# TaceoLabs/co-snarks

Hardware: NVIDIA H100
Metric: co-Groth16 proofs/sec (BN254, 2^20 constraints); MSM Mscalar/s (higher is better)
Workload: dtype u32x8 (256-bit Montgomery, integer)

## Files before the change

### co_snarks_b200/csrc/cs_curve.cuh

```cuda
#pragma once
#include "cs_field.cuh"

namespace cs {

template <class P>
struct Fp2 {
  typedef Fp<P> F;
  static constexpr int N = 2 * P::N;
  F c0, c1;
  static CS_D Fp2 zero() { Fp2 r; r.c0 = F::zero(); r.c1 = F::zero(); return r; }
  static CS_D Fp2 one() { Fp2 r; r.c0 = F::one(); r.c1 = F::zero(); return r; }
  CS_D bool is_zero() const { return c0.is_zero() && c1.is_zero(); }
  CS_D bool operator==(const Fp2& b) const { return c0 == b.c0 && c1 == b.c1; }
  CS_D bool operator!=(const Fp2& b) const { return !(*this == b); }
  friend CS_D Fp2 operator+(const Fp2& a, const Fp2& b) { Fp2 r; r.c0 = a.c0 + b.c0; r.c1 = a.c1 + b.c1; return r; }
  friend CS_D Fp2 operator-(const Fp2& a, const Fp2& b) { Fp2 r; r.c0 = a.c0 - b.c0; r.c1 = a.c1 - b.c1; return r; }
  friend CS_D Fp2 operator*(const Fp2& a, const Fp2& b) { return mul_ool(a, b); }
  static CS_DN Fp2 mul_ool(Fp2 a, Fp2 b) {
    constexpr int W = 2 * P::N;
    uint32_t v0[W], v1[W], v2[W];
    F::mul_wide(v0, a.c0, b.c0);
    F::mul_wide(v1, a.c1, b.c1);
    F::mul_wide(v2, F::add_unreduced(a.c0, a.c1), F::add_unreduced(b.c0, b.c1));
    sub_n<W>(v2, v0);
    sub_n<W>(v2, v1);
    add_mod_sq<P, 1>(v0);
    sub_n<W>(v0, v1);
    Fp2 r;
    r.c0 = F::redc(v0);
    r.c1 = F::redc(v2);
    return r;
  }
  static CS_DN Fp2 mul_sub_ool(Fp2 a, Fp2 b, Fp2 c, Fp2 d) {
    constexpr int W = 2 * P::N;
    uint32_t t0[W], t1[W], t[W];
    CS_UNROLL
    for (int i = 0; i < W; i++) t0[i] = t1[i] = mod_sq<P, 2>(i);
    F::mul_wide(t, a.c0, b.c0);
    add_n<W>(t0, t);
    sub_n<W>(t1, t);
    F::mul_wide(t, a.c1, b.c1);
    sub_n<W>(t0, t);
    sub_n<W>(t1, t);
    F::mul_wide(t, F::add_unreduced(a.c0, a.c1), F::add_unreduced(b.c0, b.c1));
    add_n<W>(t1, t);
    F::mul_wide(t, c.c0, d.c0);
    sub_n<W>(t0, t);
    add_n<W>(t1, t);
    F::mul_wide(t, c.c1, d.c1);
    add_n<W>(t0, t);
    add_n<W>(t1, t);
    F::mul_wide(t, F::add_unreduced(c.c0, c.c1), F::add_unreduced(d.c0, d.c1));
    sub_n<W>(t1, t);
    Fp2 r;
    r.c0 = F::redc(t0);
    r.c1 = F::redc(t1);
    return r;
  }
  CS_D Fp2 sqr() const { return sqr_ool(*this); }
  static CS_DN Fp2 sqr_ool(Fp2 a) {
    Fp2 r;
    F t = F::mul_inline(a.c0, a.c1);
    r.c0 = F::mul_inline(a.c0 + a.c1, a.c0 - a.c1);
    r.c1 = t + t;
    return r;
  }
  CS_D Fp2 neg() const { Fp2 r; r.c0 = c0.neg(); r.c1 = c1.neg(); return r; }
  CS_D Fp2 dbl() const { Fp2 r; r.c0 = c0.dbl(); r.c1 = c1.dbl(); return r; }
  CS_D Fp2 inverse() const {
    F n = (c0.sqr() + c1.sqr()).inverse();
    Fp2 r;
    r.c0 = c0 * n;
    r.c1 = (c1 * n).neg();
    return r;
  }
};

template <class P>
CS_D Fp<P> mul_sub(const Fp<P>& a, const Fp<P>& b, const Fp<P>& c, const Fp<P>& d) { return Fp<P>::dot2(a, b, c.neg(), d); }
template <class P>
CS_D Fp2<P> mul_sub(const Fp2<P>& a, const Fp2<P>& b, const Fp2<P>& c, const Fp2<P>& d) {
  return Fp2<P>::mul_sub_ool(a, b, c, d);
}

template <class F>
struct Affine {
  F x, y;
  CS_D bool is_inf() const { return x.is_zero() && y.is_zero(); }
  static CS_D Affine inf() { Affine r; r.x = F::zero(); r.y = F::zero(); return r; }
};

template <class F>
struct Xyzz {
  F x, y, zz, zzz;
  CS_D bool is_inf() const { return zz.is_zero(); }
  static CS_D Xyzz inf() {
    Xyzz r;
    r.x = F::zero(); r.y = F::zero(); r.zz = F::zero(); r.zzz = F::zero();
    return r;
  }
  static CS_D Xyzz from_affine(const Affine<F>& p) {
    if (p.is_inf()) return inf();
    Xyzz r;
    r.x = p.x; r.y = p.y; r.zz = F::one(); r.zzz = F::one();
    return r;
  }
};

template <class F>
CS_DN Xyzz<F> dbl_affine(const Affine<F>& p) {
  Xyzz<F> r;
  if (p.y.is_zero()) return Xyzz<F>::inf();
  F U = p.y.dbl();
  F V = U.sqr();
  F W = U * V;
  F S = p.x * V;
  F X2 = p.x.sqr();
  F M = X2.dbl() + X2;
  r.x = M.sqr() - S.dbl();
  r.y = mul_sub(M, S - r.x, W, p.y);
  r.zz = V;
  r.zzz = W;
  return r;
}

template <class F>
CS_DN Xyzz<F> dbl_xyzz(const Xyzz<F>& p) {
  if (p.is_inf() || p.y.is_zero()) return Xyzz<F>::inf();
  Xyzz<F> r;
  F U = p.y.dbl();
  F V = U.sqr();
  F W = U * V;
  F S = p.x * V;
  F X2 = p.x.sqr();
  F M = X2.dbl() + X2;
  r.x = M.sqr() - S.dbl();
  r.y = mul_sub(M, S - r.x, W, p.y);
  r.zz = V * p.zz;
  r.zzz = W * p.zzz;
  return r;
}

template <class F>
CS_D void madd(Xyzz<F>& acc, const Affine<F>& p_in, bool negate) {
  if (p_in.is_inf()) return;
  Affine<F> p = p_in;
  if (negate) p.y = p.y.neg();
  if (acc.is_inf()) {
    acc.x = p.x; acc.y = p.y; acc.zz = F::one(); acc.zzz = F::one();
    return;
  }
  F U2 = p.x * acc.zz;
  F S2 = p.y * acc.zzz;
  F Pp = U2 - acc.x;
  F R = S2 - acc.y;
  if (Pp.is_zero()) {
    if (R.is_zero()) acc = dbl_affine(p);
    else acc = Xyzz<F>::inf();
    return;
  }
  F PP = Pp.sqr();
  F PPP = Pp * PP;
  F Q = acc.x * PP;
  F X3 = R.sqr() - PPP - Q.dbl();
  acc.y = mul_sub(R, Q - X3, acc.y, PPP);
  acc.x = X3;
  acc.zz = acc.zz * PP;
  acc.zzz = acc.zzz * PPP;
}

template <class F>
CS_D void padd(Xyzz<F>& acc, const Xyzz<F>& q) {
  if (q.is_inf()) return;
  if (acc.is_inf()) { acc = q; return; }
  F U1 = acc.x * q.zz;
  F U2 = q.x * acc.zz;
  F S1 = acc.y * q.zzz;
  F S2 = q.y * acc.zzz;
  F Pp = U2 - U1;
  F R = S2 - S1;
  if (Pp.is_zero()) {
    if (R.is_zero()) acc = dbl_xyzz(acc);
    else acc = Xyzz<F>::inf();
    return;
  }
  F PP = Pp.sqr();
  F PPP = Pp * PP;
  F Q = U1 * PP;
  F X3 = R.sqr() - PPP - Q.dbl();
  acc.y = mul_sub(R, Q - X3, S1, PPP);
  acc.x = X3;
  acc.zz = acc.zz * q.zz * PP;
  acc.zzz = acc.zzz * q.zzz * PPP;
}

template <class P>
CS_D Fp<P> shfl_down(const Fp<P>& a, unsigned delta) {
  Fp<P> r;
#if defined(CS_EMU)
  cs::emu::shfl_bytes(&a, &r, sizeof(r), 1, delta);
  return r;
#endif
  CS_UNROLL
  for (int i = 0; i < P::N; i++) r.l[i] = __shfl_down_sync(0xffffffffu, a.l[i], delta);
  return r;
}
template <class P>
CS_D Fp2<P> shfl_down(const Fp2<P>& a, unsigned delta) {
  Fp2<P> r;
  r.c0 = shfl_down(a.c0, delta);
  r.c1 = shfl_down(a.c1, delta);
  return r;
}
template <class F>
CS_D Xyzz<F> shfl_down(const Xyzz<F>& p, unsigned delta) {
  Xyzz<F> r;
#if defined(CS_EMU)
  cs::emu::shfl_bytes(&p, &r, sizeof(r), 1, delta);
  return r;
#endif
  r.x = shfl_down(p.x, delta); r.y = shfl_down(p.y, delta);
  r.zz = shfl_down(p.zz, delta); r.zzz = shfl_down(p.zzz, delta);
  return r;
}

template <class F>
CS_DN Affine<F> to_affine(const Xyzz<F>& p) {
  if (p.is_inf()) return Affine<F>::inf();
  F zi = p.zzz.inverse();
  F zzi = (zi * p.zz).sqr();
  Affine<F> r;
  r.x = p.x * zzi;
  r.y = p.y * zi;
  return r;
}

}
```

### co_snarks_b200/csrc/cs_msm.cuh

```cuda
#pragma once
#include <stdlib.h>
#include "cs_common.cuh"
#include "cs_curve.cuh"

namespace cs {

constexpr unsigned MSM_SLICE_MAX = 64;
constexpr unsigned MSM_ORDER_BLOCK = 256;
constexpr unsigned MSM_RED_SEG = 4;
constexpr unsigned MSM_SIGN = 0x80000000u;

template <class FrP, class Fn>
CS_D void msm_recode(const uint32_t* __restrict__ scalars, uint32_t sstride, uint32_t i, int mont, uint32_t c,
                     uint32_t W, uint32_t k, Fn&& f) {
  Fp<FrP> s;
  const uint4* src = reinterpret_cast<const uint4*>(scalars) + (size_t)i * sstride * (FrP::N / 4);
  CS_UNROLL
  for (int q = 0; q < FrP::N / 4; q++) {
    uint4 v = src[q];
    s.l[4 * q] = v.x; s.l[4 * q + 1] = v.y; s.l[4 * q + 2] = v.z; s.l[4 * q + 3] = v.w;
  }
  if (mont) s = s.from_mont();
  const uint32_t half = 1u << (c - 1);
  const uint32_t mask = (1u << c) - 1;
  uint32_t carry = 0, row = 0, gb = 0;
  for (uint32_t w = 0; w < W; w++) {
    uint32_t pos = w * c;
    uint32_t li = pos >> 5, sh = pos & 31;
    uint32_t lo = li < FrP::N ? s.l[li] : 0;
    uint32_t hi = li + 1 < FrP::N ? s.l[li + 1] : 0;
    uint32_t d = (__funnelshift_r(lo, hi, sh) & mask) + carry;
    uint32_t out;
    if (d > half) {
      out = ((1u << c) - d) | MSM_SIGN;
      carry = 1;
    } else {
      out = d;
      carry = 0;
    }
    f(row, out & ~MSM_SIGN ? out + gb : 0);
    gb += half;
    if (gb == k * half) {
      gb = 0;
      row++;
    }
  }
}

CS_D bool msm_base_inf(const uint32_t* __restrict__ infmask, uint32_t k) {
  return infmask && ((infmask[k >> 5] >> (k & 31)) & 1);
}

constexpr unsigned MSM_BIN_T = 1024;
constexpr unsigned MSM_BIN_TILE = 4096;
constexpr unsigned MSM_BIN_SPAN = 1u << 15;
constexpr unsigned MSM_SCATTER_SPAN = 1u << 13;

template <class FrP>
CS_GLOBAL void __launch_bounds__(MSM_BIN_T) k_msm_bin_count(const uint32_t* __restrict__ scalars, uint32_t sstride,
                                                            uint32_t n, int mont, uint32_t c, uint32_t W, uint32_t kw,
                                                            const uint32_t* __restrict__ infmask, uint32_t offset,
                                                            uint32_t tile, uint32_t B, uint32_t* __restrict__ tab) {
  CS_DYN_SMEM(uint32_t, h);
  const uint32_t lo = blockIdx.y * MSM_BIN_SPAN + 1;
  const uint32_t span = B + 1 - lo < MSM_BIN_SPAN ? B + 1 - lo : MSM_BIN_SPAN;
  for (uint32_t k = threadIdx.x; k < span; k += blockDim.x) h[k] = 0;
  __syncthreads();
  const uint32_t i1 = (blockIdx.x + 1) * tile < n ? (blockIdx.x + 1) * tile : n;
  for (uint32_t i = blockIdx.x * tile + threadIdx.x; i < i1; i += blockDim.x) {
    if (msm_base_inf(infmask, offset + i)) continue;
    msm_recode<FrP>(scalars, sstride, i, mont, c, W, kw, [&](uint32_t, uint32_t d) {
      const uint32_t k = (d & ~MSM_SIGN) - lo;
      if (k < span) atomicAdd(&h[k], 1u);
    });
  }
  __syncthreads();
  uint32_t* row = tab + (size_t)blockIdx.x * B + (lo - 1);
  for (uint32_t k = threadIdx.x; k < span; k += blockDim.x) row[k] = h[k];
}

constexpr unsigned MSM_BIN_SCAN_U = 16;
static CS_GLOBAL void k_msm_bin_scan(uint32_t* __restrict__ tab, uint32_t nblk, uint32_t B, uint32_t* __restrict__ count) {
  const uint32_t b = blockIdx.x * blockDim.x + threadIdx.x;
  if (b == 0) count[0] = 0;
  if (b >= B) return;
  uint32_t* col = tab + b;
  uint32_t run = 0, r = 0;
  for (; r + MSM_BIN_SCAN_U <= nblk; r += MSM_BIN_SCAN_U) {
    uint32_t v[MSM_BIN_SCAN_U];
    CS_UNROLL
    for (uint32_t u = 0; u < MSM_BIN_SCAN_U; u++) v[u] = col[(size_t)(r + u) * B];
    CS_UNROLL
    for (uint32_t u = 0; u < MSM_BIN_SCAN_U; u++) {
      col[(size_t)(r + u) * B] = run;
      run += v[u];
    }
  }
  for (; r < nblk; r++) {
    const uint32_t v = col[(size_t)r * B];
    col[(size_t)r * B] = run;
    run += v;
  }
  count[b + 1] = run;
}

template <class FrP>
CS_GLOBAL void __launch_bounds__(MSM_BIN_T) k_msm_bin_scatter(const uint32_t* __restrict__ scalars, uint32_t sstride,
                                                              uint32_t n, int mont, uint32_t c, uint32_t W, uint32_t kw,
                                                              const uint32_t* __restrict__ infmask, uint32_t offset,
                                                              uint32_t tile, uint32_t B, uint32_t nbases,
                                                              const uint32_t* __restrict__ tab,
                                                              const uint32_t* __restrict__ start,
                                                              uint32_t* __restrict__ sorted) {
  CS_DYN_SMEM(uint32_t, cur);
  const uint32_t lo = blockIdx.y * MSM_SCATTER_SPAN + 1;
  const uint32_t span = B + 1 - lo < MSM_SCATTER_SPAN ? B + 1 - lo : MSM_SCATTER_SPAN;
  const uint32_t* row = tab + (size_t)blockIdx.x * B + (lo - 1);
  for (uint32_t k = threadIdx.x; k < span; k += blockDim.x) cur[k] = start[lo + k] + row[k];
  __syncthreads();
  const uint32_t i1 = (blockIdx.x + 1) * tile < n ? (blockIdx.x + 1) * tile : n;
  for (uint32_t i = blockIdx.x * tile + threadIdx.x; i < i1; i += blockDim.x) {
    if (msm_base_inf(infmask, offset + i)) continue;
    msm_recode<FrP>(scalars, sstride, i, mont, c, W, kw, [&](uint32_t row, uint32_t d) {
      const uint32_t k = (d & ~MSM_SIGN) - lo;
      if (k < span) sorted[atomicAdd(&cur[k], 1u)] = (row * nbases + offset + i) | (d & MSM_SIGN);
    });
  }
}

template <class F>
CS_GLOBAL void k_msm_infmask(const Affine<F>* __restrict__ table, uint32_t n, uint32_t* __restrict__ mask) {
  uint32_t wd = blockIdx.x * blockDim.x + threadIdx.x;
  if (wd * 32 >= n) return;
  uint32_t m = 0;
  for (uint32_t k = 0; k < 32 && wd * 32 + k < n; k++)
    if (table[wd * 32 + k].is_inf()) m |= 1u << k;
  mask[wd] = m;
}

constexpr unsigned MSM_SCAN_T = 1024;
constexpr unsigned MSM_SCAN_MAX_BLOCKS = 1024;
CS_D void msm_scan_terms(const uint32_t* __restrict__ count, uint32_t k, uint32_t nb1, uint32_t S, uint32_t* v) {
  uint32_t cnt = (k && k < nb1) ? count[k] : 0;
  uint32_t n0 = (cnt + S - 1) / S;
  uint32_t n1 = (n0 + S - 1) / S;
  v[0] = cnt; v[1] = n0; v[2] = n1; v[3] = (n1 + S - 1) / S;
}
static CS_GLOBAL void k_msm_scan1(const uint32_t* __restrict__ count, uint32_t nb1 , uint32_t S,
                                  uint32_t* __restrict__ start, uint32_t* __restrict__ sstart0,
                                  uint32_t* __restrict__ sstart1, uint32_t* __restrict__ sstart2, uint32_t* __restrict__ aux) {
  __shared__ uint32_t sm[4][32];
  const uint32_t t = threadIdx.x, lane = t & 31, wid = t >> 5, nwarp = blockDim.x >> 5;
  const uint32_t k = blockIdx.x * blockDim.x + t;
  uint32_t v[4], inc[4];
  msm_scan_terms(count, k, nb1, S, v);
  CS_UNROLL
  for (int q = 0; q < 4; q++) {
    uint32_t x = v[q];
    CS_UNROLL
    for (uint32_t d = 1; d < 32; d <<= 1) {
      uint32_t y = __shfl_up_sync(0xffffffffu, x, d);
      if (lane >= d) x += y;
    }
    inc[q] = x;
    if (lane == 31) sm[q][wid] = x;
  }
  __syncthreads();
  uint32_t w[4], x[4];
  CS_UNROLL
  for (int q = 0; q < 4; q++) {
    w[q] = (wid == 0 && lane < nwarp) ? sm[q][lane] : 0;
    x[q] = w[q];
    CS_UNROLL
    for (uint32_t d = 1; d < 32; d <<= 1) {
      uint32_t y = __shfl_up_sync(0xffffffffu, x[q], d);
      if (lane >= d) x[q] += y;
    }
  }
  __syncthreads();
  if (wid == 0 && lane < nwarp) {
    CS_UNROLL
    for (int q = 0; q < 4; q++) sm[q][lane] = x[q] - w[q];
    if (lane == nwarp - 1) {
      CS_UNROLL
      for (int q = 0; q < 4; q++) aux[blockIdx.x * 4 + q] = x[q];
    }
  }
  __syncthreads();
  if (k < nb1) {
    start[k] = sm[0][wid] + inc[0] - v[0];
    sstart0[k] = sm[1][wid] + inc[1] - v[1];
    sstart1[k] = sm[2][wid] + inc[2] - v[2];
    sstart2[k] = sm[3][wid] + inc[3] - v[3];
  }
}
static CS_GLOBAL void k_msm_scan2(const uint32_t* __restrict__ count, uint32_t nb1, uint32_t S,
                                  uint32_t* __restrict__ start, uint32_t* __restrict__ sstart0,
                                  uint32_t* __restrict__ sstart1, uint32_t* __restrict__ sstart2,
                                  const uint32_t* __restrict__ aux) {
  const uint32_t k = blockIdx.x * blockDim.x + threadIdx.x;
  if (k >= nb1) return;
  uint32_t off[4] = {0, 0, 0, 0};
  for (uint32_t b = 0; b < blockIdx.x; b++) {
    CS_UNROLL
    for (int q = 0; q < 4; q++) off[q] += aux[b * 4 + q];
  }
  uint32_t a = start[k] + off[0], b0 = sstart0[k] + off[1], b1 = sstart1[k] + off[2], b2 = sstart2[k] + off[3];
  start[k] = a; sstart0[k] = b0; sstart1[k] = b1; sstart2[k] = b2;
  if (k == nb1 - 1) {
    uint32_t v[4];
    msm_scan_terms(count, k, nb1, S, v);
    start[nb1] = a + v[0]; sstart0[nb1] = b0 + v[1]; sstart1[nb1] = b1 + v[2]; sstart2[nb1] = b2 + v[3];
  }
}

constexpr unsigned MSM_VIEW_T = 256;
constexpr unsigned MSM_VIEW_WORDS = MSM_VIEW_T / 32;

CS_D uint32_t popc32(uint32_t x) {
#if defined(CS_EMU)
  return (uint32_t)__builtin_popcount(x);
#else
  return __popc(x);
#endif
}
CS_D uint32_t warp_bits(bool pred) {
#if defined(CS_EMU)
  uint32_t x = pred ? 1u << (threadIdx.x & 31) : 0u;
  for (uint32_t d = 16; d > 0; d >>= 1) x += __shfl_xor_sync(0xffffffffu, x, d);
  return x;
#else
  return __ballot_sync(0xffffffffu, pred);
#endif
}

static CS_GLOBAL void k_msm_view_flags(const uint32_t* __restrict__ sorted, const uint32_t* __restrict__ src_start,
                                       uint32_t nb1, uint32_t n, const uint32_t* __restrict__ infmask, uint32_t offset,
                                       uint32_t* __restrict__ keep, uint32_t* __restrict__ blk_cnt) {
  __shared__ uint32_t cnt[MSM_VIEW_WORDS];
  const uint32_t t = threadIdx.x;
  const uint32_t p = blockIdx.x * MSM_VIEW_T + t;
  bool k = false;
  if (p < src_start[nb1]) {
    const uint32_t i = (sorted[p] & ~MSM_SIGN) % n;
    k = !((infmask[(offset + i) >> 5] >> ((offset + i) & 31)) & 1);
  }
  const uint32_t bits = warp_bits(k);
  if ((t & 31) == 0) {
    keep[(size_t)blockIdx.x * MSM_VIEW_WORDS + (t >> 5)] = bits;
    cnt[t >> 5] = popc32(bits);
  }
  __syncthreads();
  if (t == 0) {
    uint32_t c = 0;
    for (uint32_t w = 0; w < MSM_VIEW_WORDS; w++) c += cnt[w];
    blk_cnt[blockIdx.x] = c;
  }
}

static CS_GLOBAL void k_msm_view_scan(const uint32_t* __restrict__ blk_cnt, uint32_t nblk, uint32_t* __restrict__ blk_off) {
  __shared__ uint32_t sm[MSM_SCAN_T];
  const uint32_t t = threadIdx.x, T = blockDim.x;
  const uint32_t per = (nblk + T - 1) / T;
  const uint32_t lo = t * per < nblk ? t * per : nblk, hi = lo + per < nblk ? lo + per : nblk;
  uint32_t s = 0;
  for (uint32_t b = lo; b < hi; b++) s += blk_cnt[b];
  sm[t] = s;
  __syncthreads();
  for (uint32_t d = 1; d < T; d <<= 1) {
    const uint32_t v = t >= d ? sm[t - d] : 0;
    __syncthreads();
    sm[t] += v;
    __syncthreads();
  }
  uint32_t run = sm[t] - s;
  for (uint32_t b = lo; b < hi; b++) {
    const uint32_t c = blk_cnt[b];
    blk_off[b] = run;
    run += c;
  }
  if (t == T - 1) blk_off[nblk] = run;
}

CS_D uint32_t view_kept_before(uint32_t p, const uint32_t* __restrict__ keep, const uint32_t* __restrict__ blk_off) {
  const uint32_t blk = p / MSM_VIEW_T;
  uint32_t r = blk_off[blk];
  for (uint32_t w = blk * MSM_VIEW_WORDS; w < (p >> 5); w++) r += popc32(keep[w]);
  if (p & 31) r += popc32(keep[p >> 5] & ((1u << (p & 31)) - 1));
  return r;
}

static CS_GLOBAL void k_msm_view_counts(const uint32_t* __restrict__ src_start, uint32_t nb1, const uint32_t* __restrict__ keep,
                                        const uint32_t* __restrict__ blk_off, uint32_t* __restrict__ count) {
  const uint32_t b = blockIdx.x * blockDim.x + threadIdx.x;
  if (b >= nb1) return;
  count[b] = b ? view_kept_before(src_start[b + 1], keep, blk_off) - view_kept_before(src_start[b], keep, blk_off) : 0;
}

static CS_GLOBAL void k_msm_view_scatter(const uint32_t* __restrict__ sorted, uint32_t n, uint32_t nbases, uint32_t offset,
                                         const uint32_t* __restrict__ keep, const uint32_t* __restrict__ blk_off,
                                         uint32_t* __restrict__ out) {
  const uint32_t t = threadIdx.x;
  const uint32_t* kb = keep + (size_t)blockIdx.x * MSM_VIEW_WORDS;
  const uint32_t word = kb[t >> 5];
  if (!((word >> (t & 31)) & 1)) return;
  uint32_t pos = blk_off[blockIdx.x] + popc32(word & ((1u << (t & 31)) - 1));
  for (uint32_t k = 0; k < (t >> 5); k++) pos += popc32(kb[k]);
  const uint32_t e = sorted[blockIdx.x * MSM_VIEW_T + t];
  const uint32_t v = e & ~MSM_SIGN, w = v / n, i = v - w * n;
  out[pos] = (w * nbases + offset + i) | (e & MSM_SIGN);
}

CS_D uint32_t find_bucket(const uint32_t* __restrict__ arr, uint32_t nb1, uint32_t s) {
  uint32_t lo = 0, hi = nb1;
  while (hi - lo > 1) {
    uint32_t mid = (lo + hi) >> 1;
    if (arr[mid] <= s) lo = mid; else hi = mid;
  }
  return lo;
}

static CS_GLOBAL void k_msm_slice_hist(const uint32_t* __restrict__ count, const uint32_t* __restrict__ sstart0,
                                       uint32_t nb1, uint32_t S, uint32_t* __restrict__ slice_len,
                                       uint32_t* __restrict__ slice_bkt, uint32_t* __restrict__ block_hist) {
  __shared__ uint32_t h[MSM_SLICE_MAX + 1];
  for (uint32_t k = threadIdx.x; k <= MSM_SLICE_MAX; k += blockDim.x) h[k] = 0;
  __syncthreads();
  uint32_t s = blockIdx.x * blockDim.x + threadIdx.x;
  if (s < sstart0[nb1]) {
    uint32_t lo = 0, hi = nb1;
    while (hi - lo > 1) {
      uint32_t mid = (lo + hi) >> 1;
      if (sstart0[mid] <= s) lo = mid; else hi = mid;
    }
    uint32_t j = s - sstart0[lo];
    uint32_t len = count[lo] - j * S;
    if (len > S) len = S;
    slice_len[s] = len;
    slice_bkt[s] = lo;
    atomicAdd(&h[len], 1u);
  }
  __syncthreads();
  for (uint32_t k = threadIdx.x; k <= MSM_SLICE_MAX; k += blockDim.x)
    block_hist[(size_t)blockIdx.x * (MSM_SLICE_MAX + 1) + k] = h[k];
}

constexpr unsigned MSM_OFF_CHUNKS = 64;
static CS_GLOBAL void k_msm_slice_off1(const uint32_t* __restrict__ block_hist, uint32_t nblocks,
                                       uint32_t* __restrict__ chunk_sum) {
  uint32_t id = blockIdx.x * blockDim.x + threadIdx.x;
  if (id >= (MSM_SLICE_MAX + 1) * MSM_OFF_CHUNKS) return;
  uint32_t L = id / MSM_OFF_CHUNKS, ch = id % MSM_OFF_CHUNKS;
  uint32_t per = (nblocks + MSM_OFF_CHUNKS - 1) / MSM_OFF_CHUNKS;
  uint32_t lo = ch * per, hi = lo + per < nblocks ? lo + per : nblocks;
  uint32_t sum = 0;
  for (uint32_t b = lo; b < hi; b++) sum += block_hist[(size_t)b * (MSM_SLICE_MAX + 1) + L];
  chunk_sum[id] = sum;
}
static CS_GLOBAL void k_msm_slice_off2(uint32_t* __restrict__ chunk_sum, uint32_t* __restrict__ len_base) {
  uint32_t L = blockIdx.x * blockDim.x + threadIdx.x;
  if (L > MSM_SLICE_MAX) return;
  uint32_t run = 0;
  for (uint32_t c = 0; c < MSM_OFF_CHUNKS; c++) {
    uint32_t v = chunk_sum[L * MSM_OFF_CHUNKS + c];
    chunk_sum[L * MSM_OFF_CHUNKS + c] = run;
    run += v;
  }
  len_base[MSM_SLICE_MAX + 1 + L] = run;
}
static CS_GLOBAL void k_msm_slice_off3(uint32_t* __restrict__ block_hist, uint32_t nblocks,
                                       const uint32_t* __restrict__ chunk_sum, uint32_t* __restrict__ len_base) {
  uint32_t id = blockIdx.x * blockDim.x + threadIdx.x;
  if (id == 0) {
    uint32_t run = 0;
    for (int k = MSM_SLICE_MAX; k >= 0; k--) { len_base[k] = run; run += len_base[MSM_SLICE_MAX + 1 + k]; }
  }
  if (id >= (MSM_SLICE_MAX + 1) * MSM_OFF_CHUNKS) return;
  uint32_t L = id / MSM_OFF_CHUNKS, ch = id % MSM_OFF_CHUNKS;
  uint32_t per = (nblocks + MSM_OFF_CHUNKS - 1) / MSM_OFF_CHUNKS;
  uint32_t lo = ch * per, hi = lo + per < nblocks ? lo + per : nblocks;
  uint32_t run = chunk_sum[id];
  for (uint32_t b = lo; b < hi; b++) {
    uint32_t v = block_hist[(size_t)b * (MSM_SLICE_MAX + 1) + L];
    block_hist[(size_t)b * (MSM_SLICE_MAX + 1) + L] = run;
    run += v;
  }
}

static CS_GLOBAL void k_msm_slice_order(const uint32_t* __restrict__ slice_len, const uint32_t* __restrict__ slice_bkt,
                                        uint32_t nslices_max, const uint32_t* __restrict__ sstart0, uint32_t nb1,
                                        const uint32_t* __restrict__ block_off, const uint32_t* __restrict__ len_base,
                                        uint32_t* __restrict__ order, uint32_t* __restrict__ order_b) {
  __shared__ uint32_t h[MSM_SLICE_MAX + 1];
  for (uint32_t k = threadIdx.x; k <= MSM_SLICE_MAX; k += blockDim.x) h[k] = 0;
  __syncthreads();
  uint32_t s = blockIdx.x * blockDim.x + threadIdx.x;
  if (s < sstart0[nb1]) {
    uint32_t len = slice_len[s];
    uint32_t rank = atomicAdd(&h[len], 1u);
    uint32_t pos = len_base[len] + block_off[(size_t)blockIdx.x * (MSM_SLICE_MAX + 1) + len] + rank;
    order[pos] = s;
    order_b[pos] = slice_bkt[s];
  }
}

template <class F, int MINB>
CS_GLOBAL void __launch_bounds__(128, MINB) k_msm_accum0(const Affine<F>* __restrict__ table,
                                                         const uint32_t* __restrict__ sorted,
                                                         const uint32_t* __restrict__ count,
                                                         const uint32_t* __restrict__ start,
                                                         const uint32_t* __restrict__ sstart0, uint32_t nb1, uint32_t S,
                                                         const uint32_t* __restrict__ order,
                                                         const uint32_t* __restrict__ order_b,
                                                         Xyzz<F>* __restrict__ part0) {
  uint32_t t = blockIdx.x * blockDim.x + threadIdx.x;
  if (t >= sstart0[nb1]) return;
  uint32_t s = order[t];
  uint32_t b = order_b[t];
  uint32_t j = s - sstart0[b];
  uint32_t beg = start[b] + j * S;
  uint32_t end = start[b] + count[b];
  if (end > beg + S) end = beg + S;
  Xyzz<F> acc = Xyzz<F>::inf();
  uint32_t e = sorted[beg];
  if constexpr (sizeof(Affine<F>) > 64) {
    for (uint32_t k = beg; k < end; k++) {
      const uint32_t e_cur = e;
      if (k + 1 < end) {
        e = sorted[k + 1];
        prefetch_l1(table + (e & ~MSM_SIGN));
      }
      madd(acc, table[e_cur & ~MSM_SIGN], (e_cur & MSM_SIGN) != 0);
    }
    part0[s] = acc;
    return;
  }
  Affine<F> p = table[e & ~MSM_SIGN];
  for (uint32_t k = beg; k < end; k++) {
    uint32_t e_cur = e;
    Affine<F> p_cur = p;
    if (k + 1 < end) {
      e = sorted[k + 1];
      p = table[e & ~MSM_SIGN];
    }
    madd(acc, p_cur, (e_cur & MSM_SIGN) != 0);
  }
  part0[s] = acc;
}

template <class F>
CS_GLOBAL void __launch_bounds__(128) k_msm_accum1(const Xyzz<F>* __restrict__ part0,
                                                   const uint32_t* __restrict__ sstart0,
                                                   const uint32_t* __restrict__ sstart1, uint32_t nb1, uint32_t S,
                                                   Xyzz<F>* __restrict__ part1) {
  uint32_t s = blockIdx.x * blockDim.x + threadIdx.x;
  if (s >= sstart1[nb1]) return;
  uint32_t b = find_bucket(sstart1, nb1, s);
  uint32_t j = s - sstart1[b];
  uint32_t beg = sstart0[b] + j * S;
  uint32_t end = sstart0[b + 1];
  if (end > beg + S) end = beg + S;
  Xyzz<F> acc = part0[beg];
  for (uint32_t k = beg + 1; k < end; k++) padd(acc, part0[k]);
  part1[s] = acc;
}

template <class F>
CS_GLOBAL void __launch_bounds__(128) k_msm_accum2(const Xyzz<F>* __restrict__ part1,
                                                   const uint32_t* __restrict__ sstart1, uint32_t nb1,
                                                   Xyzz<F>* __restrict__ bucket) {
  uint32_t b = blockIdx.x * blockDim.x + threadIdx.x;
  if (b >= nb1) return;
  uint32_t beg = sstart1[b], end = sstart1[b + 1];
  Xyzz<F> acc = Xyzz<F>::inf();
  if (beg < end) {
    acc = part1[beg];
    for (uint32_t k = beg + 1; k < end; k++) padd(acc, part1[k]);
  }
  bucket[b] = acc;
}

template <class F>
CS_GLOBAL void __launch_bounds__(128) k_msm_reduce_seg(const Xyzz<F>* __restrict__ bucket, uint32_t NB, uint32_t B,
                                                       uint32_t L, Xyzz<F>* __restrict__ red) {
  uint32_t t = blockIdx.x * blockDim.x + threadIdx.x;
  uint32_t lo = t * L;
  if (lo >= NB) return;
  uint32_t hi = lo + L < NB ? lo + L : NB;
  const uint32_t w = lo & (B - 1);
  Xyzz<F> acc = Xyzz<F>::inf(), tot = Xyzz<F>::inf();
  for (uint32_t b = hi; b > lo; b--) {
    padd(acc, bucket[b]);
    padd(tot, acc);
  }
  if (w != 0 && !acc.is_inf()) {
    Xyzz<F> m = Xyzz<F>::inf();
    int top = 31 - __clz(w);
    for (int bit = top; bit >= 0; bit--) {
      m = dbl_xyzz(m);
      if ((w >> bit) & 1) padd(m, acc);
    }
    padd(tot, m);
  }
  red[t] = tot;
}

template <class F>
CS_GLOBAL void k_msm_final_sum(const Xyzz<F>* __restrict__ red, uint32_t cnt,
                                                      Xyzz<F>* __restrict__ out) {
  CS_DYN_SMEM(Xyzz<F>, sm);
  const uint32_t T = blockDim.x, t = threadIdx.x;
  red += (size_t)blockIdx.y * cnt;
  out += (size_t)blockIdx.y * gridDim.x;
  Xyzz<F> acc = Xyzz<F>::inf();
  for (uint32_t k = blockIdx.x * T + t; k < cnt; k += gridDim.x * T) padd(acc, red[k]);
  sm[t] = acc;
  __syncthreads();
  for (uint32_t step = T >> 1; step > 0; step >>= 1) {
    if (t < step) {
      Xyzz<F> a = sm[t];
      padd(a, sm[t + step]);
      sm[t] = a;
    }
    __syncthreads();
  }
  if (t == 0) out[blockIdx.x] = sm[0];
}

template <class F>
CS_GLOBAL void k_msm_combine_groups(const Xyzz<F>* __restrict__ gsum, uint32_t k, uint32_t c, Xyzz<F>* __restrict__ out) {
  Xyzz<F> acc = gsum[k - 1];
  for (uint32_t g = k - 1; g-- > 0;) {
    for (uint32_t d = 0; d < c; d++) acc = dbl_xyzz(acc);
    padd(acc, gsum[g]);
  }
  out[0] = acc;
}

constexpr int MSM_PRE_CHUNK = 8;
template <class F>
CS_GLOBAL void __launch_bounds__(128) k_msm_precompute(Affine<F>* __restrict__ table, uint32_t n,
                                                       uint32_t c, uint32_t W) {
  uint32_t i = blockIdx.x * blockDim.x + threadIdx.x;
  if (i >= n) return;
  Affine<F> p = table[i];
  if (p.is_inf()) {
    for (uint32_t w = 1; w < W; w++) table[(size_t)w * n + i] = Affine<F>::inf();
    return;
  }
  Xyzz<F> cur = Xyzz<F>::from_affine(p);
  uint32_t w = 1;
  while (w < W) {
    Xyzz<F> pts[MSM_PRE_CHUNK];
    F pre[MSM_PRE_CHUNK];
    int cnt = 0;
    bool degenerate = false;
    for (; cnt < MSM_PRE_CHUNK && w + cnt < W; cnt++) {
      for (uint32_t k = 0; k < c; k++) cur = dbl_xyzz(cur);
      pts[cnt] = cur;
      degenerate = degenerate || cur.is_inf();
    }
    Affine<F> last;
    if (degenerate) {
      for (int j = 0; j < cnt; j++) {
        last = to_affine(pts[j]);
        table[(size_t)(w + j) * n + i] = last;
      }
    } else {
      pre[0] = pts[0].zzz;
      for (int j = 1; j < cnt; j++) pre[j] = pre[j - 1] * pts[j].zzz;
      F inv = pre[cnt - 1].inverse();
      for (int j = cnt - 1; j >= 0; j--) {
        F zi = j ? inv * pre[j - 1] : inv;
        inv = inv * pts[j].zzz;
        F zzi = (zi * pts[j].zz).sqr();
        Affine<F> a;
        a.x = pts[j].x * zzi;
        a.y = pts[j].y * zi;
        table[(size_t)(w + j) * n + i] = a;
        if (j == cnt - 1) last = a;
      }
    }
    cur = Xyzz<F>::from_affine(last);
    w += cnt;
  }
}

template <class F, class FrP>
CS_GLOBAL void __launch_bounds__(128) k_fixed_base_mul(const Affine<F>* __restrict__ base,
                                                       const uint32_t* __restrict__ scalars, uint32_t n,
                                                       int mont, Affine<F>* __restrict__ out) {
  uint32_t i = blockIdx.x * blockDim.x + threadIdx.x;
  if (i >= n) return;
  Fp<FrP> s;
  const uint4* src = reinterpret_cast<const uint4*>(scalars) + (size_t)i * (FrP::N / 4);
  CS_UNROLL
  for (int k = 0; k < FrP::N / 4; k++) {
    uint4 v = src[k];
    s.l[4 * k] = v.x; s.l[4 * k + 1] = v.y; s.l[4 * k + 2] = v.z; s.l[4 * k + 3] = v.w;
  }
  if (mont) s = s.from_mont();
  uint32_t lim[FrP::N];
  CS_UNROLL
  for (int k = 0; k < FrP::N; k++) lim[k] = s.l[k];
  Affine<F> b = base[0];
  Xyzz<F> acc = Xyzz<F>::inf();
  for (int bit = FrP::N * 32 - 1; bit >= 0; bit--) {
    acc = dbl_xyzz(acc);
    if ((lim[bit >> 5] >> (bit & 31)) & 1) madd(acc, b, false);
  }
  out[i] = to_affine(acc);
}

struct MsmShape {
  uint32_t c, W, B;
  uint32_t k = 1, T = 0;
  uint32_t nb() const { return k * B; }
};

static inline MsmShape msm_shape(uint32_t scalar_bits, uint32_t c, uint32_t k = 1) {
  MsmShape s;
  s.c = c;
  s.W = (scalar_bits + 1 + c - 1) / c;
  s.B = 1u << (c - 1);
  s.k = k < s.W ? k : s.W;
  s.T = (s.W + s.k - 1) / s.k;
  return s;
}

static inline uint32_t msm_auto_window(size_t n, uint32_t scalar_bits) {
  int lg = 0;
  while ((1ull << (lg + 1)) <= n) lg++;
  int c = lg >= 15 ? 16 : lg - 4;
  if (c < 4) c = 4;
  while (c < 16) {
    const uint32_t W = (scalar_bits + 1 + c - 1) / c;
    const uint32_t top = scalar_bits + 1 - (W - 1) * c;
    if (2 * top >= (uint32_t)c) break;
    c++;
  }
  return (uint32_t)c;
}
static inline uint32_t msm_slice(const MsmShape& sh) {
  const char* e = getenv("CS_MSM_SLICE");
  if (e && atoi(e) == 64) return 64u;
  if (e && atoi(e) == 32) return 32u;
  return sh.c >= 18 ? 64u : 32u;
}

constexpr int MSM_NSTAGE = 5;
struct MsmWorkspace {
  DevBuf dig, sorted, meta, part0, part1, part2, bucket, red, scal, result, order;
  void* h_result = nullptr;
  size_t h_result_cap = 0;
  bool profile = false;
  cudaEvent_t ev[MSM_NSTAGE + 1] = {};
  cudaEvent_t sorted_ev = nullptr;
  bool sorted_ev_made = false, sorted_once = false;
  cudaEvent_t acc_in = nullptr, acc_out = nullptr;
  int mark(int i, cudaStream_t st) {
    if (!profile) return 0;
    if (!ev[i]) CS_CUDA(cudaEventCreateWithFlags(&ev[i], 0));
    CS_CUDA(cudaEventRecord(ev[i], st));
    return 0;
  }
  void release() {
    for (int i = 0; i <= MSM_NSTAGE; i++) {
      if (ev[i]) cudaEventDestroy(ev[i]);
      ev[i] = nullptr;
    }
    if (sorted_ev_made) cudaEventDestroy(sorted_ev);
    if (acc_in) cudaEventDestroy(acc_in);
    if (acc_out) cudaEventDestroy(acc_out);
    acc_in = acc_out = nullptr;
    sorted_ev = nullptr;
    sorted_ev_made = sorted_once = false;
    dig.release(); sorted.release(); meta.release(); part0.release(); part1.release(); part2.release();
    bucket.release(); red.release(); scal.release(); result.release(); order.release();
    if (h_result) cudaFreeHost(h_result);
    h_result = nullptr;
    h_result_cap = 0;
  }
};

template <class F>
int msm_accum0_f52(const Affine<F>* table, const uint32_t* sorted, const uint32_t* count, const uint32_t* start,
                   const uint32_t* sstart0, uint32_t nb1, uint32_t S, const uint32_t* order, const uint32_t* order_b,
                   Xyzz<F>* part0, uint32_t max_s0, cudaStream_t st);

struct MsmSizes {
  uint32_t nb1, S, ob;
  size_t nent, max_s0, max_s1, max_s2;
  MsmSizes(const MsmShape& sh, uint32_t n) {
    nb1 = sh.nb() + 1;
    nent = (size_t)sh.W * n;
    S = msm_slice(sh);
    max_s0 = nent / S + nb1;
    max_s1 = max_s0 / S + nb1;
    max_s2 = max_s1 / S + nb1;
    ob = ceil_div(max_s0, MSM_ORDER_BLOCK);
  }
  size_t meta_words() const { return (size_t)nb1 + 4 * ((size_t)nb1 + 1) + 4 * MSM_SCAN_MAX_BLOCKS; }
  size_t order_words() const {
    return 4 * max_s0 + (size_t)ob * (MSM_SLICE_MAX + 1) + 2 * (MSM_SLICE_MAX + 1) + (size_t)(MSM_SLICE_MAX + 1) * MSM_OFF_CHUNKS;
  }
};
struct MsmSortBufs {
  uint32_t *count, *start, *sstart0, *sstart1, *sstart2, *aux;
  uint32_t *slice_len, *slice_bkt, *order, *order_b, *block_hist, *len_base, *chunk_sum;
  MsmSortBufs(const MsmWorkspace& w, const MsmSizes& z) {
    count = w.meta.as<uint32_t>();
    start = count + z.nb1;
    sstart0 = start + z.nb1 + 1;
    sstart1 = sstart0 + z.nb1 + 1;
    sstart2 = sstart1 + z.nb1 + 1;
    aux = sstart2 + z.nb1 + 1;
    slice_len = w.order.as<uint32_t>();
    slice_bkt = slice_len + z.max_s0;
    order = slice_bkt + z.max_s0;
    order_b = order + z.max_s0;
    block_hist = order_b + z.max_s0;
    len_base = block_hist + (size_t)z.ob * (MSM_SLICE_MAX + 1);
    chunk_sum = len_base + 2 * (MSM_SLICE_MAX + 1);
  }
};

static inline int msm_check_limits(const MsmShape& sh, uint32_t n, uint32_t nbases) {
  const size_t nent = (size_t)sh.W * n;
  if (nent >= (1ull << 31) || (size_t)sh.T * nbases >= (1ull << 31))
    return fail(-3, "msm: W*n = %zu entries or T*nbases = %zu table slots exceed 2^31", nent, (size_t)sh.T * nbases);
  return 0;
}

static inline int msm_scan(const MsmSortBufs& q, const MsmSizes& z, uint32_t NB, cudaStream_t st) {
  const uint32_t sb = ceil_div(z.nb1, MSM_SCAN_T);
  if (sb > MSM_SCAN_MAX_BLOCKS) return fail(-3, "msm: %u buckets exceed the scan's limit", NB);
  CS_LAUNCH_SYNC(k_msm_scan1, sb, MSM_SCAN_T, 0, st, q.count, z.nb1, z.S, q.start, q.sstart0, q.sstart1, q.sstart2, q.aux);
  CS_LAUNCH(k_msm_scan2, sb, MSM_SCAN_T, 0, st, q.count, z.nb1, z.S, q.start, q.sstart0, q.sstart1, q.sstart2, q.aux);
  return 0;
}

static inline int msm_slice_order(MsmWorkspace& ws, const MsmSortBufs& q, const MsmSizes& z, cudaStream_t st) {
  CS_LAUNCH_SYNC(k_msm_slice_hist, z.ob, MSM_ORDER_BLOCK, 0, st, q.count, q.sstart0, z.nb1, z.S, q.slice_len, q.slice_bkt,
                 q.block_hist);
  const uint32_t nt = (MSM_SLICE_MAX + 1) * MSM_OFF_CHUNKS;
  CS_LAUNCH(k_msm_slice_off1, ceil_div(nt, 128), 128, 0, st, q.block_hist, z.ob, q.chunk_sum);
  CS_LAUNCH(k_msm_slice_off2, 1, 128, 0, st, q.chunk_sum, q.len_base);
  CS_LAUNCH(k_msm_slice_off3, ceil_div(nt, 128), 128, 0, st, q.block_hist, z.ob, q.chunk_sum, q.len_base);
  CS_LAUNCH_SYNC(k_msm_slice_order, z.ob, MSM_ORDER_BLOCK, 0, st, q.slice_len, q.slice_bkt, (uint32_t)z.max_s0, q.sstart0,
                 z.nb1, q.block_hist, q.len_base, q.order, q.order_b);
  if (!ws.sorted_ev_made) {
    CS_CUDA(cudaEventCreateWithFlags(&ws.sorted_ev, cudaEventDisableTiming));
    ws.sorted_ev_made = true;
  }
  CS_CUDA(cudaEventRecord(ws.sorted_ev, st));
  ws.sorted_once = true;
  return 0;
}

template <class FrP>
int msm_smem_optin() {
#if !defined(CS_EMU)
  CS_CUDA(cudaFuncSetAttribute(k_msm_bin_count<FrP>, cudaFuncAttributeMaxDynamicSharedMemorySize, MSM_BIN_SPAN * 4));
  CS_CUDA(cudaFuncSetAttribute(k_msm_bin_scatter<FrP>, cudaFuncAttributeMaxDynamicSharedMemorySize, MSM_SCATTER_SPAN * 4));
#endif
  return 0;
}

static inline uint32_t msm_bin_tile(const MsmShape& sh, const MsmSizes& z, uint32_t n) {
  const size_t rows = z.nent / sh.nb() > 1 ? z.nent / sh.nb() : 1;
  const size_t nblk = ceil_div(n, MSM_BIN_TILE) < rows ? ceil_div(n, MSM_BIN_TILE) : rows;
  return n ? ceil_div(n, nblk) : 1;
}

static inline size_t msm_sort_dig_words(const MsmShape& sh, const MsmSizes& z, uint32_t n) {
  const size_t tab_words = (size_t)(n ? ceil_div(n, msm_bin_tile(sh, z, n)) : 0) * sh.nb();
  return tab_words > z.nent ? tab_words : z.nent;
}
static inline size_t msm_view_dig_words(const MsmSizes& z) {
  const size_t nblk = ceil_div(z.nent, MSM_VIEW_T);
  return nblk * MSM_VIEW_WORDS + 2 * nblk + 1;
}

template <class F>
struct MsmReduce {
  uint32_t L, nseg_g, nseg, fs_threads, fs_blocks;
  size_t red_elems;
  explicit MsmReduce(const MsmShape& sh) {
    L = sh.B < MSM_RED_SEG ? sh.B : MSM_RED_SEG;
    nseg_g = sh.B / L;
    nseg = sh.k * nseg_g;
    fs_threads = sizeof(Xyzz<F>) > 128 ? 128 : 256;
    fs_blocks = nseg_g > 4 * fs_threads ? (nseg_g + fs_threads - 1) / fs_threads : 1;
    red_elems = (size_t)nseg + (size_t)sh.k * fs_blocks + (sh.k > 1 ? sh.k : 0);
  }
};

static inline size_t msm_sort_bytes(const MsmShape& sh, uint32_t n) {
  const MsmSizes z(sh, n);
  const size_t dig = msm_sort_dig_words(sh, z, n) > msm_view_dig_words(z) ? msm_sort_dig_words(sh, z, n) : msm_view_dig_words(z);
  return DevBuf::alloc_size(dig * 4) + DevBuf::alloc_size(z.nent * 4) + DevBuf::alloc_size(z.meta_words() * 4) +
         DevBuf::alloc_size(z.order_words() * 4);
}
template <class F>
size_t msm_accum_bytes(const MsmShape& sh, uint32_t n) {
  const MsmSizes z(sh, n);
  const size_t x = sizeof(Xyzz<F>);
  return DevBuf::alloc_size(z.max_s0 * x) + DevBuf::alloc_size(z.max_s1 * x) + DevBuf::alloc_size(z.max_s2 * x) +
         DevBuf::alloc_size((size_t)z.nb1 * x) + DevBuf::alloc_size(MsmReduce<F>(sh).red_elems * x) + DevBuf::alloc_size(x);
}

template <class FrP>
int msm_sort(MsmWorkspace& ws, const uint32_t* infmask, uint32_t nbases, MsmShape sh, uint32_t offset,
             const uint32_t* d_scalars, uint32_t sstride, uint32_t n, int mont, cudaStream_t st) {
  CS_TRY(msm_check_limits(sh, n, nbases));
  const MsmSizes z(sh, n);
  const uint32_t tile = msm_bin_tile(sh, z, n);
  const uint32_t nblk = n ? ceil_div(n, tile) : 0;
  const uint32_t NB = sh.nb();
  const dim3 grid(nblk, ceil_div(NB, MSM_BIN_SPAN)), grid_sc(nblk, ceil_div(NB, MSM_SCATTER_SPAN));
  const uint32_t smem = (NB < MSM_BIN_SPAN ? NB : MSM_BIN_SPAN) * 4;
  const uint32_t smem_sc = (NB < MSM_SCATTER_SPAN ? NB : MSM_SCATTER_SPAN) * 4;
  CS_TRY(ws.dig.reserve(msm_sort_dig_words(sh, z, n) * 4));
  CS_TRY(ws.sorted.reserve(z.nent * 4));
  CS_TRY(ws.meta.reserve(z.meta_words() * 4));
  CS_TRY(ws.order.reserve(z.order_words() * 4));
  const MsmSortBufs q(ws, z);
  uint32_t* tab = ws.dig.as<uint32_t>();
  CS_TRY(ws.mark(0, st));
  if (nblk)
    CS_LAUNCH_SYNC(k_msm_bin_count<FrP>, grid, MSM_BIN_T, smem, st, d_scalars, sstride, n, mont, sh.c, sh.W, sh.k,
                   infmask, offset, tile, NB, tab);
  CS_TRY(ws.mark(1, st));
  CS_LAUNCH(k_msm_bin_scan, ceil_div(NB, 256), 256, 0, st, tab, nblk, NB, q.count);
  CS_TRY(msm_scan(q, z, NB, st));
  if (nblk)
    CS_LAUNCH_SYNC(k_msm_bin_scatter<FrP>, grid_sc, MSM_BIN_T, smem_sc, st, d_scalars, sstride, n, mont, sh.c, sh.W, sh.k,
                   infmask, offset, tile, NB, nbases, tab, q.start, ws.sorted.as<uint32_t>());
  return msm_slice_order(ws, q, z, st);
}

static inline int msm_view(MsmWorkspace& ws, const MsmWorkspace& src, const uint32_t* infmask, uint32_t nbases,
                           MsmShape sh, uint32_t offset, uint32_t n, cudaStream_t st) {
  const MsmSizes z(sh, n);
  const uint32_t nblk = ceil_div(z.nent, MSM_VIEW_T);
  CS_TRY(ws.dig.reserve(msm_view_dig_words(z) * 4));
  CS_TRY(ws.sorted.reserve(z.nent * 4));
  CS_TRY(ws.meta.reserve(z.meta_words() * 4));
  CS_TRY(ws.order.reserve(z.order_words() * 4));
  const MsmSortBufs q(ws, z), s(src, z);
  uint32_t* keep = ws.dig.as<uint32_t>();
  uint32_t* blk_cnt = keep + (size_t)nblk * MSM_VIEW_WORDS;
  uint32_t* blk_off = blk_cnt + nblk;
  const uint32_t* src_sorted = src.sorted.as<uint32_t>();
  CS_LAUNCH_SYNC(k_msm_view_flags, nblk, MSM_VIEW_T, 0, st, src_sorted, s.start, z.nb1, n, infmask, offset, keep, blk_cnt);
  CS_LAUNCH_SYNC(k_msm_view_scan, 1, MSM_SCAN_T, 0, st, blk_cnt, nblk, blk_off);
  CS_LAUNCH(k_msm_view_counts, ceil_div(z.nb1, 256), 256, 0, st, s.start, z.nb1, keep, blk_off, q.count);
  CS_LAUNCH(k_msm_view_scatter, nblk, MSM_VIEW_T, 0, st, src_sorted, n, nbases, offset, keep, blk_off,
            ws.sorted.as<uint32_t>());
  CS_TRY(msm_scan(q, z, sh.nb(), st));
  return msm_slice_order(ws, q, z, st);
}

template <class F, class FrP>
int msm_enqueue(MsmWorkspace& ws, const Affine<F>* table, const uint32_t* infmask, uint32_t nbases, MsmShape sh,
                uint32_t offset,
                const uint32_t* d_scalars, uint32_t sstride, uint32_t n, int mont, cudaStream_t st,
                MsmWorkspace* sort_from = nullptr, bool view = false, bool table_m260 = false, cudaStream_t st_acc = nullptr) {
  CS_TRY(msm_check_limits(sh, n, nbases));
  const MsmSizes z(sh, n);
  const uint32_t nb1 = z.nb1, S = z.S;
  const size_t max_s0 = z.max_s0, max_s1 = z.max_s1, max_s2 = z.max_s2;
  CS_TRY(ws.part0.reserve(max_s0 * sizeof(Xyzz<F>)));
  CS_TRY(ws.part1.reserve(max_s1 * sizeof(Xyzz<F>)));
  CS_TRY(ws.part2.reserve(max_s2 * sizeof(Xyzz<F>)));
  CS_TRY(ws.bucket.reserve((size_t)nb1 * sizeof(Xyzz<F>)));
  const MsmReduce<F> rd(sh);
  const uint32_t L = rd.L, nseg = rd.nseg, fs_threads = rd.fs_threads, fs_blocks = rd.fs_blocks;
  CS_TRY(ws.red.reserve(rd.red_elems * sizeof(Xyzz<F>)));
  CS_TRY(ws.result.reserve(sizeof(Xyzz<F>)));
  if (ws.h_result_cap < sizeof(Xyzz<F>)) {
    if (ws.h_result) cudaFreeHost(ws.h_result);
    CS_CUDA(cudaMallocHost(&ws.h_result, sizeof(Xyzz<F>)));
    ws.h_result_cap = sizeof(Xyzz<F>);
  }
  if (sort_from) {
    if (!sort_from->sorted_once) return fail(-1, "msm: the workspace to share a sort with has not been enqueued");
    CS_TRY(ws.mark(0, st));
    CS_CUDA(cudaStreamWaitEvent(st, sort_from->sorted_ev, 0));
    CS_TRY(ws.mark(1, st));
    if (view) CS_TRY(msm_view(ws, *sort_from, infmask, nbases, sh, offset, n, st));
  } else {
    CS_TRY(msm_sort<FrP>(ws, infmask, nbases, sh, offset, d_scalars, sstride, n, mont, st));
  }
  MsmWorkspace& so = sort_from && !view ? *sort_from : ws;
  const MsmSortBufs q(so, z);
  const uint32_t *count = q.count, *start = q.start, *sstart0 = q.sstart0, *sstart1 = q.sstart1, *sstart2 = q.sstart2;
  const uint32_t *order = q.order, *order_b = q.order_b;
  CS_TRY(ws.mark(2, st));
  cudaStream_t st_main = st;
  if (st_acc) {
    if (!ws.acc_in) {
      CS_CUDA(cudaEventCreateWithFlags(&ws.acc_in, cudaEventDisableTiming));
      CS_CUDA(cudaEventCreateWithFlags(&ws.acc_out, cudaEventDisableTiming));
    }
    CS_CUDA(cudaEventRecord(ws.acc_in, st));
    CS_CUDA(cudaStreamWaitEvent(st_acc, ws.acc_in, 0));
    st = st_acc;
  }
  {
    static int minb_env = -1;
    if (minb_env < 0) { const char* e = getenv("CS_ACCUM0_MINB"); minb_env = e ? atoi(e) : 0; }
    const int minb = minb_env ? minb_env : (sizeof(Affine<F>) > 64 ? 2 : 4);
    if (table_m260) {
      CS_TRY((msm_accum0_f52<F>(table, so.sorted.as<uint32_t>(), count, start, sstart0, nb1, S, order, order_b,
                                ws.part0.as<Xyzz<F>>(), (uint32_t)max_s0, st)));
    } else {
#define CS_ACC0(M)                                                                                              \
  CS_LAUNCH(k_msm_accum0<F COMMA M>, ceil_div(max_s0, 128), 128, 0, st, table, so.sorted.as<uint32_t>(), count, \
            start, sstart0, nb1, S, order, order_b, ws.part0.as<Xyzz<F>>())
    switch (minb) {
      case 2: CS_ACC0(2); break;
      case 3: CS_ACC0(3); break;
      case 5: CS_ACC0(5); break;
      case 6: CS_ACC0(6); break;
      default: CS_ACC0(4); break;
    }
#undef CS_ACC0
    }
  }
  if (st_acc) {
    CS_CUDA(cudaEventRecord(ws.acc_out, st_acc));
    st = st_main;
    CS_CUDA(cudaStreamWaitEvent(st, ws.acc_out, 0));
  }
  CS_TRY(ws.mark(3, st));
  CS_LAUNCH(k_msm_accum1<F>, ceil_div(max_s1, 128), 128, 0, st, ws.part0.as<Xyzz<F>>(), sstart0, sstart1,
            nb1, S, ws.part1.as<Xyzz<F>>());
  CS_LAUNCH(k_msm_accum1<F>, ceil_div(max_s2, 128), 128, 0, st, ws.part1.as<Xyzz<F>>(), sstart1, sstart2,
            nb1, S, ws.part2.as<Xyzz<F>>());
  CS_LAUNCH(k_msm_accum2<F>, ceil_div(nb1, 128), 128, 0, st, ws.part2.as<Xyzz<F>>(), sstart2, nb1,
            ws.bucket.as<Xyzz<F>>());
  CS_TRY(ws.mark(4, st));
  CS_LAUNCH(k_msm_reduce_seg<F>, ceil_div(nseg, 128), 128, 0, st, ws.bucket.as<Xyzz<F>>(), sh.nb(), sh.B, L,
            ws.red.as<Xyzz<F>>());
  Xyzz<F>* gsum = sh.k > 1 ? ws.red.as<Xyzz<F>>() + nseg + (size_t)sh.k * fs_blocks : ws.result.as<Xyzz<F>>();
  if (fs_blocks > 1) {
    Xyzz<F>* stage = ws.red.as<Xyzz<F>>() + nseg;
    CS_LAUNCH_SYNC(k_msm_final_sum<F>, dim3(fs_blocks, sh.k), fs_threads, fs_threads * sizeof(Xyzz<F>), st,
                   ws.red.as<Xyzz<F>>(), rd.nseg_g, stage);
    CS_LAUNCH_SYNC(k_msm_final_sum<F>, dim3(1, sh.k), fs_threads, fs_threads * sizeof(Xyzz<F>), st, stage, fs_blocks, gsum);
  } else {
    CS_LAUNCH_SYNC(k_msm_final_sum<F>, dim3(1, sh.k), fs_threads, fs_threads * sizeof(Xyzz<F>), st, ws.red.as<Xyzz<F>>(),
                   rd.nseg_g, gsum);
  }
  if (sh.k > 1)
    CS_LAUNCH(k_msm_combine_groups<F>, 1, 1, 0, st, gsum, sh.k, sh.c, ws.result.as<Xyzz<F>>());
  CS_TRY(ws.mark(5, st));
  CS_CUDA(cudaMemcpyAsync(ws.h_result, ws.result.p, sizeof(Xyzz<F>), cudaMemcpyDeviceToHost, st));
  CS_CUDA(cudaGetLastError());
  return 0;
}

}
```

Measured before the change: 51.87.

## Split G2 bucket accumulation across thread pairs with shuffle-based mixed addition

For Fp2 (G2) points, the first-stage bucket accumulation kernel now assigns each bucket segment to two adjacent lanes. One lane holds x/zz and the other y/zzz, and they exchange intermediates through pair shuffles inside a new madd_pair routine and a split mul_sub. This halves per-thread register state for G2 so occupancy can rise (minBlocks 3), at the cost of extra shuffles, duplicated control flow and doubled thread count. The launch for the two-lane path uses a synchronous launch macro.

After: 51.70 (median of 6 runs). About the same (-0.3%).

```diff
diff --git a/co_snarks_b200/csrc/cs_curve.cuh b/co_snarks_b200/csrc/cs_curve.cuh
--- a/co_snarks_b200/csrc/cs_curve.cuh
+++ b/co_snarks_b200/csrc/cs_curve.cuh
@@ -169,6 +169,118 @@
   acc.zzz = acc.zzz * PPP;
 }
 
+#if defined(CS_EMU)
+namespace emu {
+inline void pair_swap_bytes(const void* in, void* out, size_t bytes) {
+  static std::atomic<uint32_t> seq[1024];
+  static unsigned char box[1024][512];
+  const unsigned tid = threadIdx.x + blockDim.x * (threadIdx.y + blockDim.y * threadIdx.z), other = tid ^ 1;
+  const uint32_t k = seq[tid].load(std::memory_order_relaxed);
+  memcpy(box[tid], in, bytes);
+  seq[tid].store(k + 1, std::memory_order_release);
+  while (seq[other].load(std::memory_order_acquire) < k + 1) std::this_thread::yield();
+  memcpy(out, box[other], bytes);
+  seq[tid].store(k + 2, std::memory_order_release);
+  while (seq[other].load(std::memory_order_acquire) < k + 2) std::this_thread::yield();
+}
+}
+#endif
+CS_D void pair_swap_words(const uint32_t* in, uint32_t* out, int n) {
+#if defined(CS_EMU)
+  emu::pair_swap_bytes(in, out, 4 * (size_t)n);
+#else
+  const unsigned mask = 3u << (threadIdx.x & 30);
+  CS_UNROLL
+  for (int i = 0; i < n; i++) out[i] = __shfl_xor_sync(mask, in[i], 1);
+#endif
+}
+CS_D uint32_t pair_swap(uint32_t v) {
+  uint32_t r;
+  pair_swap_words(&v, &r, 1);
+  return r;
+}
+template <class P>
+CS_D Fp<P> pair_swap(const Fp<P>& a) {
+  Fp<P> r;
+  pair_swap_words(a.l, r.l, P::N);
+  return r;
+}
+template <class P>
+CS_D Fp2<P> pair_swap(const Fp2<P>& a) {
+  Fp2<P> r;
+  r.c0 = pair_swap(a.c0);
+  r.c1 = pair_swap(a.c1);
+  return r;
+}
+
+template <class P>
+CS_DN Fp<P> mul_sub_pair(Fp2<P> x, Fp2<P> y, bool odd) {
+  typedef Fp<P> F;
+  constexpr int W = 2 * P::N;
+  uint32_t v0[W], v1[W], t[W];
+  F::mul_wide(v0, x.c0, y.c0);
+  CS_UNROLL
+  for (int i = 0; i < W; i++) v1[i] = 0;
+  sub_n<W>(v1, v0);
+  F::mul_wide(t, x.c1, y.c1);
+  sub_n<W>(v0, t);
+  sub_n<W>(v1, t);
+  F::mul_wide(t, F::add_unreduced(x.c0, x.c1), F::add_unreduced(y.c0, y.c1));
+  add_n<W>(v1, t);
+  uint32_t other[W];
+  CS_UNROLL
+  for (int i = 0; i < W; i++) t[i] = odd ? v0[i] : v1[i];
+  pair_swap_words(t, other, W);
+  CS_UNROLL
+  for (int i = 0; i < W; i++) {
+    v0[i] = odd ? other[i] : v0[i];
+    v1[i] = odd ? v1[i] : other[i];
+    t[i] = mod_sq<P, 2>(i);
+  }
+  add_n<W>(t, v1);
+  sub_n<W>(t, v0);
+  return F::redc(t);
+}
+
+template <class P>
+CS_D void madd_pair(Fp2<P>& x, Fp2<P>& z, Fp2<P> p, bool negate, bool odd) {
+  typedef Fp2<P> F;
+  uint32_t f = (p.is_zero() ? 1u : 0u) | (z.is_zero() ? 2u : 0u);
+  f |= pair_swap(f) << 2;
+  if ((f & 5) == 5) return;
+  if (odd && negate) p = p.neg();
+  if (f & (odd ? 8u : 2u)) {
+    x = p;
+    z = F::one();
+    return;
+  }
+  const F d = p * z - x;
+  uint32_t g = d.is_zero() ? 1u : 0u;
+  g |= pair_swap(g) << 1;
+  if (g & (odd ? 2u : 1u)) {
+    const F q = pair_swap(p);
+    Affine<F> a;
+    a.x = odd ? q : p;
+    a.y = odd ? p : q;
+    Xyzz<F> r = (g & 3) == 3 ? dbl_affine(a) : Xyzz<F>::inf();
+    x = odd ? r.y : r.x;
+    z = odd ? r.zzz : r.zz;
+    return;
+  }
+  const F s = d.sqr();
+  const F xo = pair_swap(x), so = pair_swap(s);
+  const F m = (odd ? xo : d) * (odd ? so : s);
+  const F y1 = odd ? x : xo;
+  const F mo = pair_swap(m);
+  const F ppp = odd ? mo : m, q = odd ? m : mo;
+  const F x3 = (odd ? s : so) - ppp - q.dbl();
+  z = z * (odd ? ppp : s);
+  const Fp<P> y = mul_sub_pair<P>(odd ? d : y1, odd ? q - x3 : ppp, odd);
+  const Fp<P> yo = pair_swap(y);
+  if (odd) { x.c0 = yo; x.c1 = y; }
+  else x = x3;
+}
+
 template <class F>
 CS_D void padd(Xyzz<F>& acc, const Xyzz<F>& q) {
   if (q.is_inf()) return;
diff --git a/co_snarks_b200/csrc/cs_msm.cuh b/co_snarks_b200/csrc/cs_msm.cuh
--- a/co_snarks_b200/csrc/cs_msm.cuh
+++ b/co_snarks_b200/csrc/cs_msm.cuh
@@ -404,6 +404,11 @@
   }
 }
 
+template <class F>
+struct Accum0Lanes { static constexpr uint32_t value = 1; };
+template <class P>
+struct Accum0Lanes<Fp2<P>> { static constexpr uint32_t value = 2; };
+
 template <class F, int MINB>
 CS_GLOBAL void __launch_bounds__(128, MINB) k_msm_accum0(const Affine<F>* __restrict__ table,
                                                          const uint32_t* __restrict__ sorted,
@@ -413,7 +418,7 @@
                                                          const uint32_t* __restrict__ order,
                                                          const uint32_t* __restrict__ order_b,
                                                          Xyzz<F>* __restrict__ part0) {
-  uint32_t t = blockIdx.x * blockDim.x + threadIdx.x;
+  uint32_t t = (blockIdx.x * blockDim.x + threadIdx.x) / Accum0Lanes<F>::value;
   if (t >= sstart0[nb1]) return;
   uint32_t s = order[t];
   uint32_t b = order_b[t];
@@ -421,8 +426,24 @@
   uint32_t beg = start[b] + j * S;
   uint32_t end = start[b] + count[b];
   if (end > beg + S) end = beg + S;
+  uint32_t e = sorted[beg];
+  if constexpr (Accum0Lanes<F>::value == 2) {
+    const bool odd = threadIdx.x & 1;
+    const F* half = reinterpret_cast<const F*>(table) + odd;
+    F x = F::zero(), z = F::zero();
+    for (uint32_t k = beg; k < end; k++) {
+      const uint32_t e_cur = e;
+      if (k + 1 < end) {
+        e = sorted[k + 1];
+        prefetch_l1(half + 2 * (e & ~MSM_SIGN));
+      }
+      madd_pair(x, z, half[2 * (e_cur & ~MSM_SIGN)], (e_cur & MSM_SIGN) != 0, odd);
+    }
+    if (odd) { part0[s].y = x; part0[s].zzz = z; }
+    else { part0[s].x = x; part0[s].zz = z; }
+    return;
+  }
   Xyzz<F> acc = Xyzz<F>::inf();
-  uint32_t e = sorted[beg];
   if constexpr (sizeof(Affine<F>) > 64) {
     for (uint32_t k = beg; k < end; k++) {
       const uint32_t e_cur = e;
@@ -911,14 +932,20 @@
   {
     static int minb_env = -1;
     if (minb_env < 0) { const char* e = getenv("CS_ACCUM0_MINB"); minb_env = e ? atoi(e) : 0; }
-    const int minb = minb_env ? minb_env : (sizeof(Affine<F>) > 64 ? 2 : 4);
+    constexpr uint32_t lanes = Accum0Lanes<F>::value;
+    const int minb = minb_env ? minb_env : (lanes == 2 ? 3 : sizeof(Affine<F>) > 64 ? 2 : 4);
+    const size_t nthreads = max_s0 * lanes;
     if (table_m260) {
       CS_TRY((msm_accum0_f52<F>(table, so.sorted.as<uint32_t>(), count, start, sstart0, nb1, S, order, order_b,
                                 ws.part0.as<Xyzz<F>>(), (uint32_t)max_s0, st)));
     } else {
-#define CS_ACC0(M)                                                                                              \
-  CS_LAUNCH(k_msm_accum0<F COMMA M>, ceil_div(max_s0, 128), 128, 0, st, table, so.sorted.as<uint32_t>(), count, \
-            start, sstart0, nb1, S, order, order_b, ws.part0.as<Xyzz<F>>())
+#define CS_ACC0(M)                                                                                                   \
+  if (lanes == 2)                                                                                                   \
+    CS_LAUNCH_SYNC(k_msm_accum0<F COMMA M>, ceil_div(nthreads, 128), 128, 0, st, table, so.sorted.as<uint32_t>(),    \
+                   count, start, sstart0, nb1, S, order, order_b, ws.part0.as<Xyzz<F>>());                           \
+  else                                                                                                               \
+    CS_LAUNCH(k_msm_accum0<F COMMA M>, ceil_div(nthreads, 128), 128, 0, st, table, so.sorted.as<uint32_t>(), count, \
+              start, sstart0, nb1, S, order, order_b, ws.part0.as<Xyzz<F>>())
     switch (minb) {
       case 2: CS_ACC0(2); break;
       case 3: CS_ACC0(3); break;
```
